# RagnarGrootKoerkamp/astar-pairwise-aligner

Measured on AMD Instinct MI355X. Metric: DP cell-updates/sec (GCUPS), full bit-parallel DP, 100kbp@5% div, higher is better.
Workload: dtype u32

## Files before the change

astar-pairwise-aligner_amd/csrc/slice_kernel.hpp:

```cpp
#pragma once
#include <hip/hip_runtime.h>
#include <stdint.h>

#include "slice_job_order.hpp"

namespace pa {
namespace slice {

#ifndef PA_SLICE_CLOCK_TURNS
#define PA_SLICE_CLOCK_TURNS 15
#endif
#ifndef PA_SLICE_YIELD
#define PA_SLICE_YIELD 2
#endif
constexpr int kPad = 64;
constexpr int kErrSpin = 7;
constexpr uint32_t kSpinLimit = 1u << 22;

struct SliceGroup {
    uint64_t a_off;
    uint64_t b_off;
    uint64_t h_off;
    uint32_t h_stride;
    int32_t n;
    int32_t nstrips;
    int32_t npairs;
    uint32_t first_pos;
    uint32_t ev_first, ev_count;
    uint32_t pad_;
};
struct SliceEvent {
    int32_t col;
    uint32_t mask;
};
struct SlicePair {
    uint64_t a_off, b_off;
    int32_t n, m;
    uint32_t pair;
    uint32_t pad_;
};

typedef uint32_t pa_slice_u32x2 __attribute__((ext_vector_type(2)));
__device__ __forceinline__ uint32_t dpp_wave_shr1(uint32_t old_, uint32_t src) {
    return (uint32_t)__builtin_amdgcn_update_dpp((int)old_, (int)src, 0x138, 0xf, 0xf, false);
}
__device__ __forceinline__ uint32_t dpp_wave_rol1(uint32_t x) {
    return (uint32_t)__builtin_amdgcn_update_dpp((int)x, (int)x, 0x134, 0xf, 0xf, false);
}
__device__ __forceinline__ uint2 ld_boundary(const uint2* p) {
    const unsigned long long v = __hip_atomic_load((const unsigned long long*)p, __ATOMIC_RELAXED, __HIP_MEMORY_SCOPE_AGENT);
    return make_uint2((uint32_t)v, (uint32_t)(v >> 32));
}
__device__ __forceinline__ void st_boundary(uint2* p, uint32_t hp, uint32_t hm) {
    __hip_atomic_store((unsigned long long*)p, (unsigned long long)hp | ((unsigned long long)hm << 32), __ATOMIC_RELAXED, __HIP_MEMORY_SCOPE_AGENT);
}

#define PA_SLICE_ROW_PAIR(vpA, vmA, vpB, vmB, nb0A, nb1A, nb0B, nb1B, a0, a1, hpp, hmp, hpo, hmo)                                      \
    do {                                                                                                                                \
        uint32_t zA_, zB_, hmA_, hpA_;                                                                                                  \
        asm volatile(                                                                                                                   \
            "v_xor_b32 %[zA], %[a1_], %[nb1A_]\n\t"                                                                                     \
            "v_xor_b32 %[zB], %[a1_], %[nb1B_]\n\t"                                                                                     \
            "v_bitop3_b32 %[zA], %[a0_], %[nb0A_], %[zA] bitop3:0x28\n\t"                                                               \
            "v_bitop3_b32 %[zB], %[a0_], %[nb0B_], %[zB] bitop3:0x28\n\t"                                                               \
            "v_bitop3_b32 %[zA], %[zA], %[vmA_], %[hmp_] bitop3:0xfe\n\t"                                                               \
            "v_and_b32 %[hmA], %[zA], %[vpA_]\n\t"                                                                                      \
            "v_bitop3_b32 %[hpA], %[vmA_], %[zA], %[vpA_] bitop3:0xf1\n\t"                                                              \
            "v_bitop3_b32 %[zB], %[zB], %[vmB_], %[hmA] bitop3:0xfe\n\t"                                                                \
            "v_bitop3_b32 %[vpA_], %[hmp_], %[zA], %[hpp_] bitop3:0xf1\n\t"                                                             \
            "v_and_b32 %[hmB], %[zB], %[vpB_]\n\t"                                                                                      \
            "v_and_b32 %[vmA_], %[hpp_], %[zA]\n\t"                                                                                     \
            "v_bitop3_b32 %[hpB], %[vmB_], %[zB], %[vpB_] bitop3:0xf1\n\t"                                                              \
            "v_bitop3_b32 %[vpB_], %[hmA], %[zB], %[hpA] bitop3:0xf1\n\t"                                                               \
            "v_and_b32 %[vmB_], %[hpA], %[zB]"                                                                                          \
            : [zA] "=&v"(zA_), [zB] "=&v"(zB_), [hmA] "=&v"(hmA_), [hpA] "=&v"(hpA_), [hmB] "=&v"(hmo), [hpB] "=&v"(hpo),              \
              [vpA_] "+v"(vpA), [vmA_] "+v"(vmA), [vpB_] "+v"(vpB), [vmB_] "+v"(vmB)                                                    \
            : [a0_] "v"(a0), [a1_] "v"(a1), [nb0A_] "v"(nb0A), [nb1A_] "v"(nb1A), [nb0B_] "v"(nb0B), [nb1B_] "v"(nb1B), [hpp_] "v"(hpp), \
              [hmp_] "v"(hmp));                                                                                                         \
    } while (0)

#define PA_SLICE_ROW_ONE(vpA, vmA, nb0A, nb1A, a0, a1, hpp, hmp, hpo, hmo)                                                              \
    do {                                                                                                                                \
        uint32_t zA_;                                                                                                                   \
        asm volatile(                                                                                                                   \
            "v_xor_b32 %[zA], %[a1_], %[nb1A_]\n\t"                                                                                     \
            "v_bitop3_b32 %[zA], %[a0_], %[nb0A_], %[zA] bitop3:0x28\n\t"                                                               \
            "v_bitop3_b32 %[zA], %[zA], %[vmA_], %[hmp_] bitop3:0xfe\n\t"                                                               \
            "v_and_b32 %[hmA], %[zA], %[vpA_]\n\t"                                                                                      \
            "v_bitop3_b32 %[hpA], %[vmA_], %[zA], %[vpA_] bitop3:0xf1\n\t"                                                              \
            "v_bitop3_b32 %[vpA_], %[hmp_], %[zA], %[hpp_] bitop3:0xf1\n\t"                                                             \
            "v_and_b32 %[vmA_], %[hpp_], %[zA]"                                                                                          \
            : [zA] "=&v"(zA_), [hmA] "=&v"(hmo), [hpA] "=&v"(hpo), [vpA_] "+v"(vpA), [vmA_] "+v"(vmA)                                   \
            : [a0_] "v"(a0), [a1_] "v"(a1), [nb0A_] "v"(nb0A), [nb1A_] "v"(nb1A), [hpp_] "v"(hpp), [hmp_] "v"(hmp));                    \
    } while (0)

constexpr int kRingEntries = 256;
constexpr uint32_t kRingMask = (uint32_t)(kRingEntries - 1) * 16u;

#define PA_SLICE_FEED(hpp, hmp, ohp, ohm, hin, min_)                                                                                     \
    asm volatile(                                                                                                                       \
        "s_mov_b64 vcc, 1\n\t"                                                                                                          \
        "v_cndmask_b32_dpp %[hpp_], %[ohp_], %[hin_], vcc wave_shr:1 row_mask:0xf bank_mask:0xf bound_ctrl:0\n\t"                       \
        "v_cndmask_b32_dpp %[hmp_], %[ohm_], %[hmin_], vcc wave_shr:1 row_mask:0xf bank_mask:0xf bound_ctrl:0"                          \
        : [hpp_] "=&v"(hpp), [hmp_] "=&v"(hmp)                                                                                          \
        : [ohp_] "v"(ohp), [ohm_] "v"(ohm), [hin_] "v"(hin), [hmin_] "v"(min_)                                                          \
        : "vcc")

template <int R>
__global__ __launch_bounds__(64, 2) void slice_kernel(const SliceJob* __restrict__ jobs, int njobs, const SliceGroup* __restrict__ groups,
                                                      const SliceEvent* __restrict__ events, const uint2* __restrict__ A, const uint2* __restrict__ B,
                                                      uint2* H, uint2* V, uint32_t* ticket_err, unsigned long long* dbg) {
    __shared__ uint4 ring[kRingEntries];
    const int lane = (int)threadIdx.x;
    const uint32_t wave_slot = (uint32_t)__builtin_amdgcn_s_getreg((4 - 1) << 11 | 4) & 15u;
    for (;;) {
        uint32_t tk = 0;
        if (lane == 0) tk = atomicAdd(ticket_err, 1u);
        tk = (uint32_t)__builtin_amdgcn_readfirstlane((int)tk);
        if (tk >= (uint32_t)njobs) break;
        const SliceJob job = jobs[tk];
        const SliceGroup grp = groups[job.group];
        const unsigned long long t_job0 = dbg ? __builtin_amdgcn_s_memrealtime() : 0ull;
        unsigned long long t_parked = 0, n_parks = 0;
        [[maybe_unused]] bool waited_before = false;
        [[maybe_unused]] int slack = 0;
        const int s = (int)job.strip, n = grp.n;
        const bool has_in = s > 0, has_out = s + 1 < grp.nstrips;
        const uint2* Ag = A + grp.a_off + kPad;
        const size_t row0 = grp.b_off + ((size_t)s * 64 + (size_t)lane) * R;
        const uint2* Hin = H + grp.h_off + (size_t)(has_in ? s - 1 : 0) * grp.h_stride + kPad;
        uint2* Hout = H + grp.h_off + (size_t)(has_out ? s : 0) * grp.h_stride + kPad;
        const SliceEvent* ev = events + grp.ev_first;
        uint32_t nb0[R], nb1[R], vp[R], vm[R];
#pragma unroll
        for (int i = 0; i < R; ++i) {
            const uint2 b = B[row0 + i];
            nb0[i] = b.x;
            nb1[i] = b.y;
            vp[i] = ~0u;
            vm[i] = 0u;
        }
        constexpr int kWaitStep = 8;
        uint32_t a0 = 0, a1 = 0, o_hp = 0, o_hm = ~0u;
        uint32_t off = (lane == 63 && has_out) ? (uint32_t)(-lane) * 8u : 0x7FFFFFF0u;
        int cnt = 1 - lane;
        int cnt16 = cnt * 16;
        constexpr int kNoEvent = INT32_MIN;
        uint32_t ev_i = 0;
        int ev_col16 = ev[0].col * 16;
        const int nchunks = (n + 63 + 63) / 64;
        const __amdgpu_buffer_rsrc_t hrs = __builtin_amdgcn_make_buffer_rsrc((void*)Hout, 0, (int)((uint32_t)n * 8u), 0x00020000);
        unsigned long long nA = 0, nH = ~0ull;
        uint2 kA = Ag[lane], kH = make_uint2(~0u, 0u);
        if (has_in) kH = ld_boundary(Hin + lane);
        ring[kRingEntries - 64 + lane] = make_uint4(0u, 0u, 0u, ~0u);
        __builtin_amdgcn_s_waitcnt(0);
        for (int q = 0; q < nchunks; ++q) {
#if PA_SLICE_CLOCK_TURNS
            if ((((uint32_t)__builtin_amdgcn_s_memrealtime() >> PA_SLICE_CLOCK_TURNS) ^ wave_slot) & 1u) __builtin_amdgcn_s_setprio(1);
            else __builtin_amdgcn_s_setprio(0);
#else
            if (((uint32_t)q ^ wave_slot) & 1u) __builtin_amdgcn_s_setprio(1);
            else __builtin_amdgcn_s_setprio(0);
#endif
            uint2 cA = kA, cH = kH;
            const int col = q * 64 + lane;
            if (has_in) {
                uint32_t spins = 0;
                const unsigned long long t_p0 = dbg ? __builtin_amdgcn_s_memrealtime() : 0ull;
                while (col < n && (cH.x & cH.y) != 0u) {
                    __builtin_amdgcn_s_sleep(32);
                    cH = ld_boundary(Hin + col);
                    if (++spins > kSpinLimit) {
                        atomicCAS(ticket_err + 1, 0u, (uint32_t)kErrSpin);
                        cH = make_uint2(~0u, 0u);
                    }
                }
                const bool waited = __builtin_amdgcn_readfirstlane((int)(__ballot(spins != 0u) != 0ull)) != 0;
#if PA_SLICE_YIELD == 1
                if (waited) __builtin_amdgcn_s_setprio(0);
#elif PA_SLICE_YIELD == 2
                if (waited || waited_before) __builtin_amdgcn_s_setprio(0);
                waited_before = waited;
#elif PA_SLICE_YIELD >= 3
                slack = waited ? PA_SLICE_YIELD : (slack > 0 ? slack - 1 : 0);
                if (slack > 0) __builtin_amdgcn_s_setprio(0);
#endif
                if (dbg && waited) {
                    t_parked += __builtin_amdgcn_s_memrealtime() - t_p0;
                    n_parks += 1;
                }
                if (col < n) st_boundary(const_cast<uint2*>(Hin) + col, ~0u, ~0u);
            }
            ring[col & (kRingEntries - 1)] = make_uint4(cA.x, cA.y, cH.x, cH.y);
            uint4 r = *(const uint4*)((const char*)ring + ((uint32_t)(cnt16 - 16) & kRingMask));
            const int pcol = min(col + 64, n + kPad - 1);
            const bool more = q + 1 < nchunks;
            if (more) {
                asm volatile("global_load_dwordx2 %0, %1, off ; pa_prefetch_load" : "=v"(nA) : "v"(Ag + pcol) : "memory");
                if (has_in) asm volatile("global_load_dwordx2 %0, %1, off sc1 ; pa_prefetch_load" : "=v"(nH) : "v"(Hin + pcol) : "memory");
            }
            const int jend = min(64, n + 63 - q * 64);
            const int wait_at = more ? kWaitStep : -1;
            for (int j = 0; j < jend; ++j) {
                asm volatile("" : "+s"(j));
                if (j == wait_at) {
                    asm volatile("s_waitcnt vmcnt(8) ; pa_prefetch_wait" : "+v"(nA), "+v"(nH)::"memory");
                    kA = make_uint2((uint32_t)nA, (uint32_t)(nA >> 32));
                    if (has_in) kH = make_uint2((uint32_t)nH, (uint32_t)(nH >> 32));
                }
                uint32_t hpp, hmp;
                a0 = r.x;
                a1 = r.y;
                PA_SLICE_FEED(hpp, hmp, o_hp, o_hm, r.z, r.w);
#pragma unroll
                for (int i = 0; i + 1 < R; i += 2) {
                    uint32_t hpo, hmo;
                    PA_SLICE_ROW_PAIR(vp[i], vm[i], vp[i + 1], vm[i + 1], nb0[i], nb1[i], nb0[i + 1], nb1[i + 1], a0, a1, hpp, hmp, hpo, hmo);
                    hpp = hpo;
                    hmp = hmo;
                }
                if constexpr (R & 1) {
                    uint32_t hpo, hmo;
                    PA_SLICE_ROW_ONE(vp[R - 1], vm[R - 1], nb0[R - 1], nb1[R - 1], a0, a1, hpp, hmp, hpo, hmo);
                    hpp = hpo;
                    hmp = hmo;
                }
                o_hp = hpp;
                o_hm = hmp;
                r = *(const uint4*)((const char*)ring + ((uint32_t)cnt16 & kRingMask));
                {
                    const pa_slice_u32x2 d = {hpp, hmp};
                    __builtin_amdgcn_raw_buffer_store_b64(d, hrs, off, 0, 16);
                }
                off += 8u;
                if (cnt16 == ev_col16) {
                    const uint32_t mask = ev[ev_i].mask;
#pragma unroll
                    for (int i = 0; i < R; ++i) {
                        atomicOr(&V[row0 + i].x, vp[i] & mask);
                        atomicOr(&V[row0 + i].y, vm[i] & mask);
                        asm volatile("" ::: "memory");
                    }
                    ++ev_i;
                    ev_col16 = ev_i < grp.ev_count ? ev[ev_i].col * 16 : kNoEvent;
                    __builtin_amdgcn_s_waitcnt(0);
                }
                cnt16 += 16;
            }
        }
        if (dbg && lane == 0) {
            const unsigned long long dt = __builtin_amdgcn_s_memrealtime() - t_job0;
            atomicMin(dbg + 0, dt);
            atomicMax(dbg + 1, dt);
            atomicAdd(dbg + 2, dt);
            atomicAdd(dbg + 3, 1ull);
            atomicAdd(dbg + 4, t_parked);
            atomicAdd(dbg + 5, n_parks);
            if (s == 0) {
                atomicMin(dbg + 6, dt);
                atomicMax(dbg + 7, dt);
            }
            const uint32_t xcc = (uint32_t)__builtin_amdgcn_s_getreg((4 - 1) << 11 | 20) & 7u;
            atomicAdd(dbg + 8 + 2 * xcc, dt - t_parked);
            atomicAdd(dbg + 9 + 2 * xcc, 1ull);
        }
    }
}


__device__ __forceinline__ uint32_t slice_rank16(const uint4 v, int count, bool& invalid) {
    const uint32_t q[4] = {v.x, v.y, v.z, v.w};
    uint32_t w = 0;
#pragma unroll
    for (int k = 0; k < 16; ++k) {
        const int r = rank_acgt((uint8_t)(q[k >> 2] >> (8 * (k & 3))));
        if (k < count) {
            invalid |= r < 0;
            w |= (uint32_t)(r & 3) << (2 * k);
        }
    }
    return w;
}

__global__ __launch_bounds__(256) void slice_pack_a_kernel(const SliceGroup* __restrict__ groups, const SlicePair* __restrict__ spairs,
                                                           const uint8_t* __restrict__ a_cat, uint2* __restrict__ A, uint32_t* __restrict__ bad) {
    const SliceGroup grp = groups[blockIdx.y];
    const int lane = (int)(threadIdx.x & 63), q = (int)(blockIdx.x * 4 + (threadIdx.x >> 6));
    if ((long long)q * 32 >= (long long)grp.n) return;
    const int p = lane & 31, half = lane >> 5, c0 = 32 * q + 16 * half;
    uint32_t w = 0;
    bool invalid = false;
    if (p < grp.npairs) {
        const SlicePair sp = spairs[grp.first_pos + p];
        if (c0 < sp.n) w = slice_rank16(*(const uint4*)(a_cat + sp.a_off + c0), sp.n - c0, invalid);
    }
    if (invalid) atomicOr(bad, 1u);
    uint32_t a0 = 0, a1 = 0;
#pragma unroll
    for (int k = 0; k < 16; ++k) {
        const unsigned long long b0 = __ballot((w >> (2 * k)) & 1u), b1 = __ballot((w >> (2 * k + 1)) & 1u);
        if ((lane & 15) == k) {
            a0 = (lane & 16) ? (uint32_t)(b0 >> 32) : (uint32_t)b0;
            a1 = (lane & 16) ? (uint32_t)(b1 >> 32) : (uint32_t)b1;
        }
    }
    const int c = q * 32 + lane;
    if (lane < 32 && c < grp.n) A[grp.a_off + kPad + c] = make_uint2(a0, a1);
}

__global__ __launch_bounds__(256) void slice_pack_b_kernel(const SliceGroup* __restrict__ groups, const SlicePair* __restrict__ spairs,
                                                           const uint8_t* __restrict__ b_cat, uint2* __restrict__ B, int rows_per_strip,
                                                           uint32_t* __restrict__ bad) {
    const SliceGroup grp = groups[blockIdx.y];
    const int lane = (int)(threadIdx.x & 63), j = (int)(blockIdx.x * 4 + (threadIdx.x >> 6));
    if ((long long)j * 64 >= (long long)grp.nstrips * rows_per_strip) return;
    const int p = lane & 31, half = lane >> 5;
    const long long r0 = (long long)j * 64 + 32 * half;
    uint32_t x0 = 0, x1 = 0;
    bool invalid = false;
    if (p < grp.npairs) {
        const SlicePair sp = spairs[grp.first_pos + p];
#pragma unroll
        for (int h = 0; h < 2; ++h) {
            const long long r = r0 + 16 * h;
            if (r < (long long)sp.m) {
                const int count = (int)min((long long)sp.m - r, 16ll);
                const uint32_t w = slice_rank16(*(const uint4*)(b_cat + sp.b_off + r), count, invalid);
                const uint32_t real = count >= 16 ? ~0u : (1u << (2 * count)) - 1u, nw = ~w & real;
                uint32_t e = 0, o = 0;
#pragma unroll
                for (int k = 0; k < 16; ++k) {
                    e |= ((nw >> (2 * k)) & 1u) << k;
                    o |= ((nw >> (2 * k + 1)) & 1u) << k;
                }
                x0 |= e << (16 * h);
                x1 |= o << (16 * h);
            }
        }
    }
    if (invalid) atomicOr(bad, 1u);
    uint32_t nb0 = 0, nb1 = 0;
#pragma unroll
    for (int k = 0; k < 32; ++k) {
        const unsigned long long b0 = __ballot((x0 >> k) & 1u), b1 = __ballot((x1 >> k) & 1u);
        if ((lane & 31) == k) {
            nb0 = half ? (uint32_t)(b0 >> 32) : (uint32_t)b0;
            nb1 = half ? (uint32_t)(b1 >> 32) : (uint32_t)b1;
        }
    }
    B[grp.b_off + (size_t)j * 64 + lane] = make_uint2(nb0, nb1);
}

constexpr int kScoreSpan = 4096;
__global__ __launch_bounds__(64) void slice_score_kernel(const SliceGroup* __restrict__ groups, const SlicePair* __restrict__ spairs,
                                                         const uint2* __restrict__ V, int32_t* __restrict__ cost_out) {
    const SliceGroup grp = groups[blockIdx.x];
    const int lane = (int)threadIdx.x;
    int my_m = 0, my_n = 0;
    uint32_t my_pair = 0;
    if (lane < grp.npairs) {
        const SlicePair sp = spairs[grp.first_pos + lane];
        my_m = sp.m;
        my_n = sp.n;
        my_pair = sp.pair;
    }
    int max_m = my_m;
#pragma unroll
    for (int o = 32; o > 0; o >>= 1) max_m = max(max_m, __shfl_xor(max_m, o));
    const int lo = (int)blockIdx.y * kScoreSpan, hi = min(max_m, lo + kScoreSpan);
    if (lo >= max_m) return;
    int acc = blockIdx.y == 0 ? my_n : 0;
    for (int r0 = lo; r0 < hi; r0 += 64) {
        const int r = r0 + lane;
        uint2 v = make_uint2(0u, 0u);
        if (r < hi) v = V[grp.b_off + r];
        for (int p = 0; p < grp.npairs; ++p) {
            const int mp = __shfl(my_m, p);
            const bool in = r < mp;
            const int pos = __popcll(__ballot(in && ((v.x >> p) & 1u))), neg = __popcll(__ballot(in && ((v.y >> p) & 1u)));
            if (lane == p) acc += pos - neg;
        }
    }
    if (lane < grp.npairs && acc != 0) atomicAdd(&cost_out[my_pair], acc);
}

}
}
```

astar-pairwise-aligner_amd/csrc/slice_plan.hpp:

```cpp
#pragma once
#include <hip/hip_runtime.h>

#include <cstddef>
#include <cstdint>

namespace pa {
namespace slice {

struct Plan;

constexpr int kRowsPerLane[] = {52, 51, 50, 49, 48, 47, 46, 45, 44, 42, 40, 36, 32, 28};

int choose_rows_per_lane(const size_t* a_len, const size_t* b_len, size_t pairs, double simds, double* est_ns);

Plan* create(const size_t* a_len, const size_t* b_len, size_t pairs, const size_t* a_off, const size_t* b_off, int rows_per_lane);
void destroy(Plan* p);

int run(Plan* p, hipStream_t s, const uint8_t* d_a, const uint8_t* d_b, uint32_t* d_bad, int32_t* d_costs, uint32_t* d_ticket_err, hipEvent_t ev0,
        hipEvent_t ev1);
void mark_clean(Plan* p);

struct Info {
    int rows_per_lane;
    size_t groups, jobs;
    int chain;
    double valu_instructions;
    double computed_rows_cells;
    double device_bytes;
    double boundary_bytes;
};
Info info(const Plan* p);
constexpr int kStepOverheadInstr = 6;

}
}
```

astar-pairwise-aligner_amd/csrc/slice_unit.hip:

```cpp
#include "slice_plan.hpp"

#include <algorithm>
#include <cmath>
#include <cstdio>
#include <cstdlib>
#include <memory>
#include <numeric>
#include <vector>

#include "pa_hip_internal.hpp"
#include "slice_kernel.hpp"

namespace pa {
namespace slice {

struct Plan {
    int R = 52;
    size_t pairs = 0;
    std::vector<SliceGroup> groups;
    std::vector<SliceJob> jobs;
    size_t a_elems = 0, b_elems = 0, h_elems = 0;
    unsigned max_col_blocks = 0, max_row_blocks = 0;
    double valu = 0, computed = 0;
    int chain = 0;
    bool h_dirty = false;
    DeviceBuf d_groups, d_events, d_jobs, d_spairs, d_A, d_B, d_V, d_H;
};

static int strips_for(size_t m, int R) { return (int)((m + (size_t)64 * R - 1) / ((size_t)64 * R)); }

static constexpr double kNsPerRowStep = 16.2, kNsStepOverhead = 11.6, kChainPenalty = 0.0015;

static constexpr int kDefaultChain = 1;
static int chain_setting() {
    const char* e = getenv("PA_SLICE_CHAIN");
    return e && *e ? std::max(0, atoi(e)) : kDefaultChain;
}
static int chain_in_flight(int chain, size_t slots, size_t ngroups, int longest) {
    return chain == 0 ? longest : std::min(std::max(chain, auto_chain(ngroups, longest, slots)), longest);
}

int choose_rows_per_lane(const size_t* a_len, const size_t* b_len, size_t pairs, double simds, double* est_ns) {
    if (const char* e = getenv("PA_SLICE")) {
        if (atoi(e) == 0) return 0;
    }
    size_t live = 0;
    for (size_t i = 0; i < pairs; ++i) {
        live += a_len[i] > 0 && b_len[i] > 0;
        if (a_len[i] >= (size_t(1) << 27) - 64 || b_len[i] >= (size_t(1) << 27)) return 0;
    }
    const bool forced = getenv("PA_SLICE") && atoi(getenv("PA_SLICE")) > 0;
    if ((live + 31) / 32 > 65535) return 0;
    if (live < 64 && !forced) return 0;
    std::vector<uint32_t> order;
    for (size_t i = 0; i < pairs; ++i)
        if (a_len[i] > 0 && b_len[i] > 0) order.push_back((uint32_t)i);
    std::sort(order.begin(), order.end(), [&](uint32_t x, uint32_t y) { return a_len[x] != a_len[y] ? a_len[x] < a_len[y] : (b_len[x] != b_len[y] ? b_len[x] < b_len[y] : x < y); });
    int best_r = 0;
    double best = -1;
    const double slots = simds * 2.0;
    for (const int R : kRowsPerLane) {
        if (forced && atoi(getenv("PA_SLICE")) > 1 && atoi(getenv("PA_SLICE")) != R) continue;
        double work = 0, longest = 0, jobs = 0;
        const size_t ngroups = (order.size() + 31) / 32;
        size_t m_max = 0;
        for (const uint32_t i : order) m_max = std::max(m_max, b_len[i]);
        const int S_max = strips_for(m_max, R);
        const int C = chain_in_flight(chain_setting(), (size_t)slots, ngroups, S_max);
        for (size_t g = 0; g * 32 < order.size(); ++g) {
            size_t n = 0, m = 0;
            for (size_t t = g * 32; t < std::min(order.size(), g * 32 + 32); ++t) {
                n = std::max(n, a_len[order[t]]);
                m = std::max(m, b_len[order[t]]);
            }
            const int S = strips_for(m, R);
            const double per_strip = ((double)n + 63.0) * (R * kNsPerRowStep + kNsStepOverhead) * (1.0 + kChainPenalty * (std::min(S, C) - 1));
            work += per_strip * S;
            jobs += S;
            longest = std::max(longest, per_strip + 128.0 * (S - 1) * (R * kNsPerRowStep + kNsStepOverhead));
        }
        const double waves = std::min(jobs, slots);
        const double speed = waves <= simds ? 1.165 : 1.0 + 0.165 * (slots - waves) / simds;
        const double rounds = jobs > slots ? std::ceil(jobs / slots) * (work / jobs) : work / waves;
        const double t = std::max(longest / 1.165, rounds / speed);
        if (best < 0 || t < best) {
            best = t;
            best_r = R;
        }
    }
    if (est_ns) *est_ns = best;
    return best_r;
}

Plan* create(const size_t* a_len, const size_t* b_len, size_t pairs, const size_t* a_off, const size_t* b_off, int rows_per_lane) {
    auto p = std::make_unique<Plan>();
    p->R = rows_per_lane;
    p->pairs = pairs;
    const int R = rows_per_lane;
    std::vector<uint32_t> order;
    for (size_t i = 0; i < pairs; ++i)
        if (a_len[i] > 0 && b_len[i] > 0) order.push_back((uint32_t)i);
    std::sort(order.begin(), order.end(), [&](uint32_t x, uint32_t y) { return a_len[x] != a_len[y] ? a_len[x] < a_len[y] : (b_len[x] != b_len[y] ? b_len[x] < b_len[y] : x < y); });
    std::vector<SlicePair> spairs(order.size());
    std::vector<SliceEvent> events;
    size_t a_at = 0, b_at = 0, h_at = 0;
    size_t max_n = 0, max_rows = 0;
    const size_t ngroups = (order.size() + 31) / 32;
    for (size_t gi = 0; gi < ngroups; ++gi) {
        const size_t g = ngroups - 1 - gi;
        SliceGroup grp{};
        grp.first_pos = (uint32_t)(g * 32);
        grp.npairs = (int32_t)std::min<size_t>(32, order.size() - g * 32);
        size_t n = 0, m = 0;
        for (int t = 0; t < grp.npairs; ++t) {
            const uint32_t i = order[g * 32 + t];
            n = std::max(n, a_len[i]);
            m = std::max(m, b_len[i]);
            spairs[g * 32 + t] = SlicePair{(uint64_t)a_off[i], (uint64_t)b_off[i], (int32_t)a_len[i], (int32_t)b_len[i], i, 0u};
        }
        grp.n = (int32_t)n;
        grp.nstrips = strips_for(m, R);
        grp.a_off = a_at;
        grp.b_off = b_at;
        grp.h_off = h_at;
        grp.h_stride = (uint32_t)(n + 2 * kPad);
        a_at += n + 2 * kPad;
        b_at += (size_t)grp.nstrips * 64 * R;
        h_at += (size_t)(grp.nstrips - 1) * grp.h_stride;
        grp.ev_first = (uint32_t)events.size();
        for (int t = 0; t < grp.npairs; ++t) {
            const int32_t col = (int32_t)a_len[order[g * 32 + t]];
            if (events.size() > grp.ev_first && events.back().col == col) events.back().mask |= 1u << t;
            else events.push_back(SliceEvent{col, 1u << t});
        }
        grp.ev_count = (uint32_t)events.size() - grp.ev_first;
        max_n = std::max(max_n, n);
        max_rows = std::max(max_rows, (size_t)grp.nstrips * 64 * R);
        p->valu += (double)grp.nstrips * ((double)n + 63.0) * (7.0 * R + kStepOverheadInstr);
        p->computed += (double)grp.nstrips * 64.0 * R * (double)n * 32.0;
        p->groups.push_back(grp);
    }
    {
        std::vector<int> nstrips;
        for (const SliceGroup& g : p->groups) nstrips.push_back(g.nstrips);
        const size_t slots = (size_t)device_cus() * 8;
        p->chain = chain_setting();
        p->jobs = job_order(nstrips, slots, p->chain);
    }
    p->a_elems = a_at;
    p->b_elems = b_at;
    p->h_elems = h_at;
    p->max_col_blocks = (unsigned)((max_n + 127) / 128);
    p->max_row_blocks = (unsigned)((max_rows / 64 + 3) / 4);
    if (p->groups.empty()) return p.release();
    if (events.empty()) events.push_back(SliceEvent{0, 0});
    if (!p->d_groups.alloc(p->groups.size() * sizeof(SliceGroup)) || !p->d_events.alloc(events.size() * sizeof(SliceEvent)) ||
        !p->d_jobs.alloc(p->jobs.size() * sizeof(SliceJob)) || !p->d_spairs.alloc(spairs.size() * sizeof(SlicePair)) || !p->d_A.alloc(a_at * 8) ||
        !p->d_B.alloc(b_at * 8) || !p->d_V.alloc(b_at * 8) || !p->d_H.alloc(std::max<size_t>(h_at, 8) * 8))
        return nullptr;
    if (!hip_ok(hipMemcpy(p->d_groups.ptr, p->groups.data(), p->groups.size() * sizeof(SliceGroup), hipMemcpyHostToDevice), "H2D slice groups") ||
        !hip_ok(hipMemcpy(p->d_events.ptr, events.data(), events.size() * sizeof(SliceEvent), hipMemcpyHostToDevice), "H2D slice events") ||
        !hip_ok(hipMemcpy(p->d_jobs.ptr, p->jobs.data(), p->jobs.size() * sizeof(SliceJob), hipMemcpyHostToDevice), "H2D slice jobs") ||
        !hip_ok(hipMemcpy(p->d_spairs.ptr, spairs.data(), spairs.size() * sizeof(SlicePair), hipMemcpyHostToDevice), "H2D slice pairs") ||
        !hip_ok(hipMemset(p->d_A.ptr, 0, a_at * 8), "memset slice A") ||
        (h_at && !hip_ok(hipMemset(p->d_H.ptr, 0xFF, h_at * 8), "memset slice boundaries")))
        return nullptr;
    return p.release();
}

void destroy(Plan* p) { delete p; }

void mark_clean(Plan* p) { p->h_dirty = false; }

template <int R>
static hipError_t launch_slice(int grid, hipStream_t s, const Plan* p, uint32_t* d_ticket_err, unsigned long long* dbg) {
    hipLaunchKernelGGL((slice_kernel<R>), dim3((unsigned)grid), dim3(64), 0, s, p->d_jobs.as<SliceJob>(), (int)p->jobs.size(), p->d_groups.as<SliceGroup>(),
                       p->d_events.as<SliceEvent>(), p->d_A.as<uint2>(), p->d_B.as<uint2>(), p->d_H.as<uint2>(), p->d_V.as<uint2>(), d_ticket_err, dbg);
    return hipGetLastError();
}

int run(Plan* p, hipStream_t s, const uint8_t* d_a, const uint8_t* d_b, uint32_t* d_bad, int32_t* d_costs, uint32_t* d_ticket_err, hipEvent_t ev0,
        hipEvent_t ev1) {
    if (!hip_ok(hipMemsetAsync(d_ticket_err, 0, 8, s), "memset slice ticket")) return PA_E_HIP;
    if (p->groups.empty()) {
        if (ev0 && (!hip_ok(hipEventRecord(ev0, s), "event") || !hip_ok(hipEventRecord(ev1, s), "event"))) return PA_E_HIP;
        return 0;
    }
    const unsigned G = (unsigned)p->groups.size();
    hipLaunchKernelGGL(slice_pack_a_kernel, dim3(p->max_col_blocks, G), dim3(256), 0, s, p->d_groups.as<SliceGroup>(), p->d_spairs.as<SlicePair>(), d_a,
                       p->d_A.as<uint2>(), d_bad);
    hipLaunchKernelGGL(slice_pack_b_kernel, dim3(p->max_row_blocks, G), dim3(256), 0, s, p->d_groups.as<SliceGroup>(), p->d_spairs.as<SlicePair>(), d_b,
                       p->d_B.as<uint2>(), 64 * p->R, d_bad);
    if (!hip_ok(hipGetLastError(), "slice transposes")) return PA_E_HIP;
    if (!hip_ok(hipMemsetAsync(p->d_V.ptr, 0, p->b_elems * 8, s), "memset slice V")) return PA_E_HIP;
    if (p->h_elems && p->h_dirty && !hip_ok(hipMemsetAsync(p->d_H.ptr, 0xFF, p->h_elems * 8, s), "memset slice boundaries")) return PA_E_HIP;
    p->h_dirty = true;
    int grid = (int)std::min<size_t>(p->jobs.size(), (size_t)device_cus() * 8);
    const int grid_cap = getenv("PA_SLICE_GRID") ? atoi(getenv("PA_SLICE_GRID")) : 0;
    if (grid_cap > 0) grid = std::min(grid, grid_cap);
    static const bool jobtimes = getenv("PA_SLICE_JOBTIMES") != nullptr;
    unsigned long long* dbg = nullptr;
    if (jobtimes && hipMalloc((void**)&dbg, 192) == hipSuccess) {
        const unsigned long long init[24] = {~0ull, 0, 0, 0, 0, 0, ~0ull, 0};
        if (hipMemcpyAsync(dbg, init, 192, hipMemcpyHostToDevice, s) != hipSuccess || hipStreamSynchronize(s) != hipSuccess) dbg = nullptr;
    }
    if (ev0 && !hip_ok(hipEventRecord(ev0, s), "event")) return PA_E_HIP;
    hipError_t e = hipSuccess;
    switch (p->R) {
        case 52: e = launch_slice<52>(grid, s, p, d_ticket_err, dbg); break;
        case 51: e = launch_slice<51>(grid, s, p, d_ticket_err, dbg); break;
        case 50: e = launch_slice<50>(grid, s, p, d_ticket_err, dbg); break;
        case 49: e = launch_slice<49>(grid, s, p, d_ticket_err, dbg); break;
        case 48: e = launch_slice<48>(grid, s, p, d_ticket_err, dbg); break;
        case 47: e = launch_slice<47>(grid, s, p, d_ticket_err, dbg); break;
        case 46: e = launch_slice<46>(grid, s, p, d_ticket_err, dbg); break;
        case 45: e = launch_slice<45>(grid, s, p, d_ticket_err, dbg); break;
        case 44: e = launch_slice<44>(grid, s, p, d_ticket_err, dbg); break;
        case 42: e = launch_slice<42>(grid, s, p, d_ticket_err, dbg); break;
        case 40: e = launch_slice<40>(grid, s, p, d_ticket_err, dbg); break;
        case 36: e = launch_slice<36>(grid, s, p, d_ticket_err, dbg); break;
        case 32: e = launch_slice<32>(grid, s, p, d_ticket_err, dbg); break;
        case 28: e = launch_slice<28>(grid, s, p, d_ticket_err, dbg); break;
        default: set_error("slice: no kernel for %d rows per lane", p->R); return PA_E_INTERNAL;
    }
    if (!hip_ok(e, "slice_kernel")) return PA_E_HIP;
    if (ev1 && !hip_ok(hipEventRecord(ev1, s), "event")) return PA_E_HIP;
    if (dbg) {
        unsigned long long h[24] = {0};
        if (hipMemcpyAsync(h, dbg, 192, hipMemcpyDeviceToHost, s) == hipSuccess && hipStreamSynchronize(s) == hipSuccess && h[3]) {
            std::fprintf(stderr, "[slice jobs] awake us per job by XCD:");
            for (int x = 0; x < 8; ++x) std::fprintf(stderr, " %d: %.0f (%llu)", x, h[9 + 2 * x] ? h[8 + 2 * x] * 0.01 / (double)h[9 + 2 * x] : 0.0, h[9 + 2 * x]);
            std::fprintf(stderr, "\n");
            std::fprintf(stderr, "[slice jobs] R %d chain %d: %llu jobs, us per job: min %.1f mean %.1f max %.1f (first strips: min %.1f max %.1f); asleep behind the strip above: %.2f %% of the job time, %.1f waits per job\n",
                         p->R, p->chain, h[3], h[0] * 0.01, h[2] * 0.01 / (double)h[3], h[1] * 0.01, h[6] * 0.01, h[7] * 0.01, 100.0 * (double)h[4] / (double)h[2], (double)h[5] / (double)h[3]);
        }
        (void)hipFree(dbg);
    }
    hipLaunchKernelGGL(slice_score_kernel, dim3(G, (p->max_row_blocks * 256u + kScoreSpan - 1) / kScoreSpan), dim3(64), 0, s, p->d_groups.as<SliceGroup>(), p->d_spairs.as<SlicePair>(), p->d_V.as<uint2>(), d_costs);
    if (!hip_ok(hipGetLastError(), "slice_score_kernel")) return PA_E_HIP;
    return 0;
}

Info info(const Plan* p) {
    Info i{};
    i.rows_per_lane = p->R;
    i.groups = p->groups.size();
    i.jobs = p->jobs.size();
    i.chain = p->chain;
    i.valu_instructions = p->valu;
    i.computed_rows_cells = p->computed;
    i.device_bytes = (double)(p->a_elems + 2 * p->b_elems + p->h_elems) * 8.0;
    i.boundary_bytes = (double)p->h_elems * 8.0;
    return i;
}

}
}
```

Baseline: 274,500.

## Split inner DP loop into segments to hoist per-step event and wait checks

Restructures the per-chunk inner loop into segments computed from step index, prefetch-wait position and the currently open event window. Inside a segment the tight loop carries no per-step checks for the prefetch wait or the event column, and the waitcnt is issued only around event-window steps. The planner cost model's per-step overhead constants are lowered to match. The risk is extra branching at segment boundaries, and the event-window logic is subtle and could mis-time the V atomics.

```diff
diff --git a/astar-pairwise-aligner_amd/csrc/slice_kernel.hpp b/astar-pairwise-aligner_amd/csrc/slice_kernel.hpp
--- a/astar-pairwise-aligner_amd/csrc/slice_kernel.hpp
+++ b/astar-pairwise-aligner_amd/csrc/slice_kernel.hpp
@@ -3,6 +3,7 @@
 #include <stdint.h>
 
 #include "slice_job_order.hpp"
+#include "slice_segments.hpp"
 
 namespace pa {
 namespace slice {
@@ -140,75 +141,79 @@
             vp[i] = ~0u;
             vm[i] = 0u;
         }
-        constexpr int kWaitStep = 8;
         uint32_t a0 = 0, a1 = 0, o_hp = 0, o_hm = ~0u;
         uint32_t off = (lane == 63 && has_out) ? (uint32_t)(-lane) * 8u : 0x7FFFFFF0u;
         int cnt = 1 - lane;
         int cnt16 = cnt * 16;
         constexpr int kNoEvent = INT32_MIN;
         uint32_t ev_i = 0;
-        int ev_col16 = ev[0].col * 16;
-        const int nchunks = (n + 63 + 63) / 64;
+        int ev_col16 = ev[0].col * 16 + 16;
+        uint32_t open_i = 0;
+        int32_t open_col = ev[0].col;
+        const auto ev_col_at = [ev](uint32_t i) { return ev[i].col; };
+        const int steps = job_steps(n);
         const __amdgpu_buffer_rsrc_t hrs = __builtin_amdgcn_make_buffer_rsrc((void*)Hout, 0, (int)((uint32_t)n * 8u), 0x00020000);
         unsigned long long nA = 0, nH = ~0ull;
         uint2 kA = Ag[lane], kH = make_uint2(~0u, 0u);
         if (has_in) kH = ld_boundary(Hin + lane);
         ring[kRingEntries - 64 + lane] = make_uint4(0u, 0u, 0u, ~0u);
+        uint4 r = make_uint4(0u, 0u, 0u, ~0u);
         __builtin_amdgcn_s_waitcnt(0);
-        for (int q = 0; q < nchunks; ++q) {
+        for (int t = 0; t < steps;) {
+            const Segment seg = segment_at(t, n, open_col);
+            if (seg.chunk_top) {
 #if PA_SLICE_CLOCK_TURNS
-            if ((((uint32_t)__builtin_amdgcn_s_memrealtime() >> PA_SLICE_CLOCK_TURNS) ^ wave_slot) & 1u) __builtin_amdgcn_s_setprio(1);
-            else __builtin_amdgcn_s_setprio(0);
+                if ((((uint32_t)__builtin_amdgcn_s_memrealtime() >> PA_SLICE_CLOCK_TURNS) ^ wave_slot) & 1u) __builtin_amdgcn_s_setprio(1);
+                else __builtin_amdgcn_s_setprio(0);
 #else
-            if (((uint32_t)q ^ wave_slot) & 1u) __builtin_amdgcn_s_setprio(1);
-            else __builtin_amdgcn_s_setprio(0);
+                if (((uint32_t)(t >> 6) ^ wave_slot) & 1u) __builtin_amdgcn_s_setprio(1);
+                else __builtin_amdgcn_s_setprio(0);
 #endif
-            uint2 cA = kA, cH = kH;
-            const int col = q * 64 + lane;
-            if (has_in) {
-                uint32_t spins = 0;
-                const unsigned long long t_p0 = dbg ? __builtin_amdgcn_s_memrealtime() : 0ull;
-                while (col < n && (cH.x & cH.y) != 0u) {
-                    __builtin_amdgcn_s_sleep(32);
-                    cH = ld_boundary(Hin + col);
-                    if (++spins > kSpinLimit) {
-                        atomicCAS(ticket_err + 1, 0u, (uint32_t)kErrSpin);
-                        cH = make_uint2(~0u, 0u);
+                uint2 cA = kA, cH = kH;
+                const int col = t + lane;
+                if (has_in) {
+                    uint32_t spins = 0;
+                    const unsigned long long t_p0 = dbg ? __builtin_amdgcn_s_memrealtime() : 0ull;
+                    while (col < n && (cH.x & cH.y) != 0u) {
+                        __builtin_amdgcn_s_sleep(32);
+                        cH = ld_boundary(Hin + col);
+                        if (++spins > kSpinLimit) {
+                            atomicCAS(ticket_err + 1, 0u, (uint32_t)kErrSpin);
+                            cH = make_uint2(~0u, 0u);
+                        }
                     }
-                }
-                const bool waited = __builtin_amdgcn_readfirstlane((int)(__ballot(spins != 0u) != 0ull)) != 0;
+                    const bool waited = __builtin_amdgcn_readfirstlane((int)(__ballot(spins != 0u) != 0ull)) != 0;
 #if PA_SLICE_YIELD == 1
-                if (waited) __builtin_amdgcn_s_setprio(0);
+                    if (waited) __builtin_amdgcn_s_setprio(0);
 #elif PA_SLICE_YIELD == 2
-                if (waited || waited_before) __builtin_amdgcn_s_setprio(0);
-                waited_before = waited;
+                    if (waited || waited_before) __builtin_amdgcn_s_setprio(0);
+                    waited_before = waited;
 #elif PA_SLICE_YIELD >= 3
-                slack = waited ? PA_SLICE_YIELD : (slack > 0 ? slack - 1 : 0);
-                if (slack > 0) __builtin_amdgcn_s_setprio(0);
+                    slack = waited ? PA_SLICE_YIELD : (slack > 0 ? slack - 1 : 0);
+                    if (slack > 0) __builtin_amdgcn_s_setprio(0);
 #endif
-                if (dbg && waited) {
-                    t_parked += __builtin_amdgcn_s_memrealtime() - t_p0;
-                    n_parks += 1;
-                }
-                if (col < n) st_boundary(const_cast<uint2*>(Hin) + col, ~0u, ~0u);
-            }
-            ring[col & (kRingEntries - 1)] = make_uint4(cA.x, cA.y, cH.x, cH.y);
-            uint4 r = *(const uint4*)((const char*)ring + ((uint32_t)(cnt16 - 16) & kRingMask));
-            const int pcol = min(col + 64, n + kPad - 1);
-            const bool more = q + 1 < nchunks;
-            if (more) {
-                asm volatile("global_load_dwordx2 %0, %1, off ; pa_prefetch_load" : "=v"(nA) : "v"(Ag + pcol) : "memory");
-                if (has_in) asm volatile("global_load_dwordx2 %0, %1, off sc1 ; pa_prefetch_load" : "=v"(nH) : "v"(Hin + pcol) : "memory");
-            }
-            const int jend = min(64, n + 63 - q * 64);
-            const int wait_at = more ? kWaitStep : -1;
-            for (int j = 0; j < jend; ++j) {
-                asm volatile("" : "+s"(j));
-                if (j == wait_at) {
-                    asm volatile("s_waitcnt vmcnt(8) ; pa_prefetch_wait" : "+v"(nA), "+v"(nH)::"memory");
-                    kA = make_uint2((uint32_t)nA, (uint32_t)(nA >> 32));
-                    if (has_in) kH = make_uint2((uint32_t)nH, (uint32_t)(nH >> 32));
-                }
+                    if (dbg && waited) {
+                        t_parked += __builtin_amdgcn_s_memrealtime() - t_p0;
+                        n_parks += 1;
+                    }
+                    if (col < n) st_boundary(const_cast<uint2*>(Hin) + col, ~0u, ~0u);
+                }
+                ring[col & (kRingEntries - 1)] = make_uint4(cA.x, cA.y, cH.x, cH.y);
+                r = *(const uint4*)((const char*)ring + ((uint32_t)(cnt16 - 16) & kRingMask));
+                const int pcol = min(col + 64, n + kPad - 1);
+                if (seg.more) {
+                    asm volatile("global_load_dwordx2 %0, %1, off ; pa_prefetch_load" : "=v"(nA) : "v"(Ag + pcol) : "memory");
+                    if (has_in) asm volatile("global_load_dwordx2 %0, %1, off sc1 ; pa_prefetch_load" : "=v"(nH) : "v"(Hin + pcol) : "memory");
+                }
+            }
+            if (seg.wait) {
+                asm volatile("s_waitcnt vmcnt(8) ; pa_prefetch_wait" : "+v"(nA), "+v"(nH)::"memory");
+                kA = make_uint2((uint32_t)nA, (uint32_t)(nA >> 32));
+                if (has_in) kH = make_uint2((uint32_t)nH, (uint32_t)(nH >> 32));
+            }
+            int left = seg.end - t;
+            do {
+                asm volatile("" : "+s"(left));
                 uint32_t hpp, hmp;
                 a0 = r.x;
                 a1 = r.y;
@@ -234,6 +239,10 @@
                     __builtin_amdgcn_raw_buffer_store_b64(d, hrs, off, 0, 16);
                 }
                 off += 8u;
+                cnt16 += 16;
+            } while (--left != 0);
+            t = seg.end;
+            if (seg.in_window) {
                 if (cnt16 == ev_col16) {
                     const uint32_t mask = ev[ev_i].mask;
 #pragma unroll
@@ -243,11 +252,11 @@
                         asm volatile("" ::: "memory");
                     }
                     ++ev_i;
-                    ev_col16 = ev_i < grp.ev_count ? ev[ev_i].col * 16 : kNoEvent;
-                    __builtin_amdgcn_s_waitcnt(0);
-                }
-                cnt16 += 16;
-            }
+                    ev_col16 = ev_i < grp.ev_count ? ev[ev_i].col * 16 + 16 : kNoEvent;
+                }
+                __builtin_amdgcn_s_waitcnt(0);
+            }
+            skip_closed_events(t, open_i, grp.ev_count, open_col, ev_col_at);
         }
         if (dbg && lane == 0) {
             const unsigned long long dt = __builtin_amdgcn_s_memrealtime() - t_job0;
diff --git a/astar-pairwise-aligner_amd/csrc/slice_plan.hpp b/astar-pairwise-aligner_amd/csrc/slice_plan.hpp
--- a/astar-pairwise-aligner_amd/csrc/slice_plan.hpp
+++ b/astar-pairwise-aligner_amd/csrc/slice_plan.hpp
@@ -30,7 +30,7 @@
     double boundary_bytes;
 };
 Info info(const Plan* p);
-constexpr int kStepOverheadInstr = 6;
+constexpr int kStepOverheadInstr = 5;
 
 }
 }
diff --git a/astar-pairwise-aligner_amd/csrc/slice_segments.hpp b/astar-pairwise-aligner_amd/csrc/slice_segments.hpp
--- /dev/null
+++ b/astar-pairwise-aligner_amd/csrc/slice_segments.hpp
@@ -0,0 +1,46 @@
+#pragma once
+#include <cstdint>
+
+namespace pa {
+namespace slice {
+
+constexpr int32_t kWaitStep = 8;
+constexpr int32_t kNoOpenEvent = INT32_MAX / 2;
+
+struct Segment {
+    int32_t end;
+    bool chunk_top;
+    bool more;
+    bool wait;
+    bool in_window;
+};
+
+constexpr int32_t job_steps(int32_t n) { return n + 63; }
+
+constexpr bool window_closed(int32_t t, int32_t col) { return t > col + 62; }
+
+template <class ColAt>
+constexpr void skip_closed_events(int32_t t, uint32_t& ei, uint32_t count, int32_t& col, ColAt col_at) {
+    while (ei < count && window_closed(t, col)) {
+        ++ei;
+        col = ei < count ? col_at(ei) : kNoOpenEvent;
+    }
+}
+
+constexpr Segment segment_at(int32_t t, int32_t n, int32_t open_col) {
+    const int32_t last = job_steps(n), j = t & 63, next_top = t - j + 64;
+    Segment s{};
+    s.chunk_top = j == 0;
+    s.more = next_top < last;
+    s.wait = s.more && j == kWaitStep;
+    s.in_window = t >= open_col - 1;
+    int32_t end = next_top < last ? next_top : last;
+    if (s.more && j < kWaitStep) end = t - j + kWaitStep;
+    if (s.in_window) end = t + 1;
+    else if (open_col - 1 < end) end = open_col - 1;
+    s.end = end;
+    return s;
+}
+
+}
+}
diff --git a/astar-pairwise-aligner_amd/csrc/slice_unit.hip b/astar-pairwise-aligner_amd/csrc/slice_unit.hip
--- a/astar-pairwise-aligner_amd/csrc/slice_unit.hip
+++ b/astar-pairwise-aligner_amd/csrc/slice_unit.hip
@@ -29,7 +29,7 @@
 
 static int strips_for(size_t m, int R) { return (int)((m + (size_t)64 * R - 1) / ((size_t)64 * R)); }
 
-static constexpr double kNsPerRowStep = 16.2, kNsStepOverhead = 11.6, kChainPenalty = 0.0015;
+static constexpr double kNsPerRowStep = 16.2, kNsStepOverhead = 7.8, kChainPenalty = 0.0015;
 
 static constexpr int kDefaultChain = 1;
 static int chain_setting() {
```

Result: no change. 275,900 (median of 6 runs) (+0.5%).
